# CU-Production/simple_mmd_renderer

Hardware: AMD Instinct MI355X
Metric: skinned vertices/sec (instance-sharded crowd); achieved HBM GB/s vs roofline (higher is better)
Workload: dtype f32

## Files before the change

simple_mmd_renderer_amd/csrc/kernels.hip:

```cpp
#include "instance_list.hpp"
#include "kernels.hpp"
#include "motion_blend.hpp"
#include "motion_clock.hpp"

#include <type_traits>
#ifdef PK_STAMPS
#include <algorithm>
#include <cstdio>
#include <vector>
#endif

#ifdef MMDX_FAST_MATH
#pragma clang fp contract(fast)
#define MMDX_K(name) name##_fast
#else
#define MMDX_K(name) name
#endif

#if (defined(PK_SKIP_WALK) || defined(PK_SKIP_SKIN) || defined(FUSED4_SKIP_WALK) || defined(PK_STAMPS)) && !defined(MMDX_DIAGNOSTIC_BUILD)
#error "PK_SKIP_* / FUSED4_SKIP_WALK / PK_STAMPS are timing diagnostics (wrong results): add MMDX_DIAGNOSTIC_BUILD to MMDX_BUILD_DEFS"
#endif

namespace mmdx {
namespace {
// ... 14 lines not shown
#define MMDX_STORE_POLICY 1
#endif
#if MMDX_STORE_POLICY != 0 && MMDX_STORE_POLICY != 1
#error "MMDX_STORE_POLICY: 0 (plain) or 1 (nt); the inline-asm sc0/sc1 flavours of round 3 corrupted data and no longer exist"
#endif
#ifndef MMDX_WALK_ZPAIR
#define MMDX_WALK_ZPAIR 1
#endif
typedef float v4f __attribute__((ext_vector_type(4)));
__device__ __forceinline__ void store16(float4 *dst, const float4 v) {
#if MMDX_STORE_POLICY == 1
    __builtin_nontemporal_store(v4f{v.x, v.y, v.z, v.w}, reinterpret_cast<v4f *>(dst));
#else
    *dst = v;
#endif
}
__device__ __forceinline__ void store3(float *dst, float x, float y, float z) {
#if MMDX_STORE_POLICY == 1
    __builtin_nontemporal_store(x, dst); __builtin_nontemporal_store(y, dst + 1); __builtin_nontemporal_store(z, dst + 2);
#else
    dst[0] = x; dst[1] = y; dst[2] = z;
#endif
}
template <typename T>
__device__ __forceinline__ void store_elem(T *dst, const T v) {
#if MMDX_STORE_POLICY == 1
    __builtin_nontemporal_store(v, dst);
#else
    *dst = v;
#endif
}

typedef float v2f __attribute__((ext_vector_type(2)));

struct M12 {
    v2f p0, p1, p2, p3;
    v2f q0, q1;
};

__device__ __forceinline__ M12 load_m12(const float4 *P, uint32_t b) {
    const float4 A = P[b], B = P[b + 1], C = P[b + 2];
    M12 m;
    m.p0 = v2f{A.x, A.y}; m.p1 = v2f{A.z, A.w};
    m.p2 = v2f{B.x, B.y}; m.p3 = v2f{B.z, B.w};
    m.q0 = v2f{C.x, C.y}; m.q1 = v2f{C.z, C.w};
    return m;
}
__device__ __forceinline__ M12 blend2(const M12 &a, const M12 &b, float s1, float l) {
    M12 r;
    r.p0 = a.p0 * s1 + b.p0 * l; r.p1 = a.p1 * s1 + b.p1 * l;
    r.p2 = a.p2 * s1 + b.p2 * l; r.p3 = a.p3 * s1 + b.p3 * l;
    r.q0 = a.q0 * s1 + b.q0 * l; r.q1 = a.q1 * s1 + b.q1 * l;
    return r;
}
__device__ __forceinline__ M12 mul_add(const M12 &a, float wa, const M12 &b, float wb) {
    M12 r;
    r.p0 = a.p0 * wa + b.p0 * wb; r.p1 = a.p1 * wa + b.p1 * wb;
    r.p2 = a.p2 * wa + b.p2 * wb; r.p3 = a.p3 * wa + b.p3 * wb;
    r.q0 = a.q0 * wa + b.q0 * wb; r.q1 = a.q1 * wa + b.q1 * wb;
    return r;
}
__device__ __forceinline__ M12 add_mul(const M12 &t, const M12 &c, float wc) {
    M12 r;
    r.p0 = t.p0 + c.p0 * wc; r.p1 = t.p1 + c.p1 * wc;
    r.p2 = t.p2 + c.p2 * wc; r.p3 = t.p3 + c.p3 * wc;
    r.q0 = t.q0 + c.q0 * wc; r.q1 = t.q1 + c.q1 * wc;
    return r;
}
__device__ __forceinline__ void xform_pos(const M12 &m, v2f xy, float z, v2f &oxy, float &oz) {
    oxy = ((m.p0 * xy.x + m.p1 * xy.y) + m.p2 * z) + m.p3;
    const v2f t = m.q0 * xy;
    oz = ((t.x + t.y) + z * m.q1.x) + m.q1.y;
}
__device__ __forceinline__ void xform_nrm(const M12 &m, v2f xy, float z, v2f &oxy, float &oz) {
    oxy = (m.p0 * xy.x + m.p1 * xy.y) + m.p2 * z;
    const v2f t = m.q0 * xy;
    oz = (t.x + t.y) + z * m.q1.x;
}

template <typename T>
__device__ __forceinline__ void copy_chunk(const unsigned char *img, T *g, uint32_t q, uint32_t shift,
                                           uint32_t n, bool aligned16) {
    constexpr uint32_t EPC = 16 / sizeof(T);
    const uint32_t lo = q * EPC;
    if (aligned16 && lo >= shift && lo + EPC <= shift + n) {
        const float4 v = *reinterpret_cast<const float4 *>(img + size_t(q) * 16);
        store16(reinterpret_cast<float4 *>(g + lo), v);
    } else {
        const T *l = reinterpret_cast<const T *>(img);
#pragma unroll
        for (uint32_t e = 0; e < EPC; ++e) {
            const uint32_t i = lo + e;
            if (i >= shift && i < shift + n) store_elem(g + i, l[i]);
        }
    }
}

template <int THREADS, typename TA, typename TB>
__device__ __forceinline__ void copy_out2(const unsigned char *imgA, TA *outA, size_t baseA,
                                          uint32_t shA, uint32_t nA, const unsigned char *imgB,
                                          TB *outB, size_t baseB, uint32_t shB, uint32_t nB,
                                          bool aligned16, int tid) {
    const uint32_t ncA = (shA + nA + 16 / sizeof(TA) - 1) / (16 / sizeof(TA));
    const uint32_t ncB = (shB + nB + 16 / sizeof(TB) - 1) / (16 / sizeof(TB));
    TA *gA = outA + baseA - shA;
    TB *gB = outB + baseB - shB;
    for (uint32_t q = tid; q < ncA + ncB; q += THREADS) {
        if (q < ncA) copy_chunk<TA>(imgA, gA, q, shA, nA, aligned16);
        else copy_chunk<TB>(imgB, gB, q - ncA, shB, nB, aligned16);
    }
}


template <int THREADS, int CA, int CB, int I, bool WT = false>
struct CopyFast {
    static __device__ __forceinline__ void run(const unsigned char *img, uint32_t gapB, float4 *outA,
                                               float4 *outB, int tid) {
        constexpr int TOTAL = CA + CB;
        if constexpr (I * THREADS < TOTAL) {
            constexpr bool full = (I + 1) * THREADS <= TOTAL;
            const int q = tid + I * THREADS;
            const bool inA = (I + 1) * THREADS <= CA ? true : (I * THREADS >= CA ? false : q < CA);
            float4 v = make_float4(0.f, 0.f, 0.f, 0.f);
            if (full || q < TOTAL)
                v = *reinterpret_cast<const float4 *>(img + (inA ? 0u : gapB - uint32_t(CA) * 16u) +
                                                      size_t(q) * 16);
            CopyFast<THREADS, CA, CB, I + 1, WT>::run(img, gapB, outA, outB, tid);
            if (full || q < TOTAL) {
                if constexpr (WT) {
                    typedef unsigned int v4u __attribute__((ext_vector_type(4)));
                    constexpr int kSc1Nt = 2 | 16;
                    const v4u d = {__float_as_uint(v.x), __float_as_uint(v.y), __float_as_uint(v.z), __float_as_uint(v.w)};
                    if (inA) {
                        const __amdgpu_buffer_rsrc_t r = __builtin_amdgcn_make_buffer_rsrc(outA, 0, uint32_t(CA) * 16u, 0x00027000);
                        __builtin_amdgcn_raw_buffer_store_b128(d, r, uint32_t(q) * 16u, 0, kSc1Nt);
                    } else {
                        const __amdgpu_buffer_rsrc_t r = __builtin_amdgcn_make_buffer_rsrc(outB, 0, uint32_t(CB) * 16u, 0x00027000);
                        __builtin_amdgcn_raw_buffer_store_b128(d, r, uint32_t(q - CA) * 16u, 0, kSc1Nt);
                    }
                } else {
                    float4 *dst = inA ? outA + q : outB + (q - CA);
                    store16(dst, v);
                }
            }
        }
    }
};
template <int THREADS, int CA, int CB, bool WT = false>
__device__ __forceinline__ void copy_out_fast(const unsigned char *img, uint32_t gapB, float4 *outA,
                                              float4 *outB, int tid) {
    CopyFast<THREADS, CA, CB, 0, WT>::run(img, gapB, outA, outB, tid);
}

struct Slot {
    v2f pxy, nxy, uv;
    float pz, nz;
    float w0, w1, w2, w3;
    uint32_t b0, b1, b2, b3;
    uint32_t perm;
    uint32_t rb, rlen;
    int cls;
    bool act;
};

template <bool F16>
struct RawEntry { using type = float4; };
template <>
struct RawEntry<true> { using type = uint2; };

constexpr uint32_t kRowAhead = 4;

template <bool F16, uint32_t B = kRowAhead>
struct RowHead {
    typename RawEntry<F16>::type e[B];
};
template <bool F16>
__device__ __forceinline__ typename RawEntry<F16>::type row_entry(const void *entries, uint32_t base, uint32_t j) {
    using Raw = typename RawEntry<F16>::type;
    const uint32_t off = (base + j * 64u) * uint32_t(sizeof(Raw));
    return *reinterpret_cast<const Raw *>(static_cast<const unsigned char *>(entries) + off);
}
template <bool F16, uint32_t B = kRowAhead>
__device__ __forceinline__ void row_prefetch(const void *entries, uint32_t base, uint32_t len, RowHead<F16, B> &h) {
    using Raw = typename RawEntry<F16>::type;
    const uint32_t last = len ? len - 1 : 0u;
#pragma unroll
    for (uint32_t i = 0; i < B; ++i) {
        Raw v = Raw{};
        if (len) v = row_entry<F16>(entries, base, min(i, last));
        h.e[i] = v;
    }
}
template <bool F16, uint32_t B = kRowAhead, typename Body>
__device__ __forceinline__ void row_consume(const void *entries, uint32_t base, uint32_t len, const RowHead<F16, B> &h,
                                            Body body) {
    using Raw = typename RawEntry<F16>::type;
    auto apply = [&](const Raw r) {
        if constexpr (F16) {
            body(h2f(r.x & 0xffffu), h2f(r.x >> 16), h2f(r.y & 0xffffu), uint32_t(r.y >> 16));
        } else {
            body(r.x, r.y, r.z, __float_as_uint(r.w));
        }
    };
    if (len == 0) return;
    const uint32_t last = len - 1;
    Raw cur[B], nxt[B];
#pragma unroll
    for (uint32_t i = 0; i < B; ++i) cur[i] = h.e[i];
    for (uint32_t j = 0; j < len; j += B) {
#pragma unroll
        for (uint32_t i = 0; i < B; ++i) nxt[i] = cur[i];
        if (j + B < len) {
#pragma unroll
            for (uint32_t i = 0; i < B; ++i) nxt[i] = row_entry<F16>(entries, base, min(j + B + i, last));
        }
#pragma unroll
        for (uint32_t i = 0; i < B; ++i)
            if (i == 0 || j + i < len) apply(cur[i]);
#pragma unroll
        for (uint32_t i = 0; i < B; ++i) cur[i] = nxt[i];
    }
}
template <bool F16, uint32_t B = kRowAhead, typename Body>
__device__ __forceinline__ void for_row(const void *entries, uint32_t base, uint32_t len, Body body) {
    RowHead<F16, B> h;
    row_prefetch<F16, B>(entries, base, len, h);
    row_consume<F16, B>(entries, base, len, h, body);
}

#ifndef MMDX_WALK_DEPTH32
#define MMDX_WALK_DEPTH32 4
#endif
#ifndef MMDX_WALK_DEPTH16
#define MMDX_WALK_DEPTH16 4
#endif
template <bool F16>
struct WalkHead {
    static constexpr uint32_t D = F16 ? MMDX_WALK_DEPTH16 : MMDX_WALK_DEPTH32;
    typename RawEntry<F16>::type e[D];
};
template <bool F16>
__device__ __forceinline__ void walk_head(const void *entries, uint32_t base, uint32_t len, WalkHead<F16> &h) {
    using Raw = typename RawEntry<F16>::type;
    const uint32_t last = len ? len - 1 : 0u;
#pragma unroll
    for (uint32_t i = 0; i < WalkHead<F16>::D; ++i) h.e[i] = len ? row_entry<F16>(entries, base, min(i, last)) : Raw{};
}
template <bool F16, typename Body>
__device__ __forceinline__ void walk_from_head(const void *entries, uint32_t base, uint32_t len, WalkHead<F16> &h, Body body) {
    using Raw = typename RawEntry<F16>::type;
    constexpr uint32_t D = WalkHead<F16>::D;
    if (len == 0) return;
    auto apply = [&](const Raw r) {
        if constexpr (F16) body(h2f(r.x & 0xffffu), h2f(r.x >> 16), h2f(r.y & 0xffffu), uint32_t(r.y >> 16));
        else body(r.x, r.y, r.z, __float_as_uint(r.w));
    };
    const uint32_t last = len - 1;
    uint32_t j = 0;
    for (; j + D < len; j += D) {
#pragma unroll
        for (uint32_t i = 0; i < D; ++i) {
            apply(h.e[i]);
            h.e[i] = row_entry<F16>(entries, base, min(j + D + i, last));
        }
    }
#pragma unroll
    for (uint32_t i = 0; i < D; ++i)
        if (i == 0 || j + i < len) apply(h.e[i]);
}
template <bool F16, typename Body>
__device__ __forceinline__ void walk_rolling(const void *entries, uint32_t base, uint32_t len, Body body) {
    WalkHead<F16> h;
    walk_head<F16>(entries, base, len, h);
    walk_from_head<F16>(entries, base, len, h, body);
}

__device__ __forceinline__ float slot_weight(const float *rates, const uint32_t *slot_top,
                                             const uint32_t *chain_off, const float *chain_rate,
                                             uint32_t s) {
    float r = rates[slot_top[s]];
    bool skip = r < kMorphEps;
    for (uint32_t c = chain_off[s]; !skip && c < chain_off[s + 1]; ++c) {
        r = chain_rate[c] * r;
        skip = r < kMorphEps;
    }
    return skip ? 0.f : r;
}

__device__ __forceinline__ bool map_workgroup(const DeformParams &p, uint32_t &tile, uint32_t &grp) {
    const uint32_t xcd = blockIdx.x & 7u, k = blockIdx.x >> 3;
    const uint32_t T = p.ntiles >> 3, main_count = T * p.ngroups;
    if (k < main_count) {
        grp = k / T;
        tile = xcd * T + (k - grp * T);
        return true;
    }
    const uint32_t r = xcd * p.rem_per_xcd + (k - main_count);
    if (r >= (p.ntiles & 7u) * p.ngroups) return false;
    const uint32_t rt = r / p.ngroups;
    tile = 8u * T + rt;
    grp = r - rt * p.ngroups;
    return true;
}

template <int LAYOUT, int MORPH, bool F16>
__device__ __forceinline__ void load_slot(const DeformParams &p, const TileHdr &th, uint32_t s, Slot &q) {
// ... 87 lines not shown
    const bool flat = p.fused_rates == nullptr;
    auto row_src = [&](uint32_t e, uint32_t bone) {
        const uint32_t g = gcount == 1 ? 0u : e / nb4;
        uint32_t inst = inst0 + g * istep;
        if constexpr (SEL) {
            inst = p.sel_ids[inst];
            if (inst >= p.ni) inst = 0u;
        }
        return reinterpret_cast<const float4 *>(p.palettes + size_t(inst) * p.nb * 16 + size_t(bone) * 16 + (e & 3u) * 4);
    };
    auto row_put = [&](uint32_t e, const float4 row) {
        const uint32_t g = gcount == 1 ? 0u : e / nb4, rem = e - g * nb4, lb = rem >> 2, r = rem & 3u;
        float *en = reinterpret_cast<float *>(pal + size_t(g) * p.pal_stride) + lb * 12;
        *reinterpret_cast<float2 *>(en + (r >> 1) * 4 + (r & 1u) * 2) = make_float2(row.x, row.y);
        en[8 + r] = row.z;
    };
    auto chain = [&](float r, uint32_t c0, uint32_t c1) {
        bool skip = r < kMorphEps;
        for (uint32_t c = c0; !skip && c < c1; ++c) {
            r = p.chain_rate[c] * r;
            skip = r < kMorphEps;
        }
        return skip ? 0.f : r;
    };

#pragma unroll
    for (int k = 0; k < VPT; ++k) load_slot<LAYOUT, MORPH, F16>(p, th, slot_base + uint32_t(tid) + uint32_t(k) * THREADS, sl[k]);
    uint32_t bone[kPalBatch];
#pragma unroll
    for (int i = 0; i < kPalBatch; ++i) {
        const uint32_t e = uint32_t(tid) + uint32_t(i) * THREADS;
        bone[i] = e < rows ? bones[((gcount == 1 ? e : e % nb4)) >> 2] : 0u;
    }
    uint32_t top[kWgtBatch], c0[kWgtBatch], c1[kWgtBatch];
    float wv[kWgtBatch];
#pragma unroll
    for (int i = 0; i < kWgtBatch; ++i) {
        const uint32_t sidx = uint32_t(tid) + uint32_t(i) * THREADS;
        top[i] = c0[i] = c1[i] = 0u;
        wv[i] = 0.f;
        if (kWalk && sidx < ns) {
            if (flat) wv[i] = p.wslot[sidx];
            else { top[i] = p.slot_top[sidx]; c0[i] = p.chain_off[sidx]; c1[i] = p.chain_off[sidx + 1]; }
        }
    }
    if constexpr (kWalk) {
#pragma unroll
        for (int k = 0; k < VPT; ++k) row_prefetch<F16, BH>(p.entries, sl[k].rb, sl[k].rlen, hd[k]);
    }
    float4 row[kPalBatch];
#pragma unroll
    for (int i = 0; i < kPalBatch; ++i) {
        const uint32_t e = uint32_t(tid) + uint32_t(i) * THREADS;
        row[i] = e < rows ? *row_src(e, bone[i]) : make_float4(0.f, 0.f, 0.f, 0.f);
    }
    if (kWalk && !flat) {
#pragma unroll
        for (int i = 0; i < kWgtBatch; ++i)
            if (uint32_t(tid) + uint32_t(i) * THREADS < ns) wv[i] = p.fused_rates[top[i]];
    }
#pragma unroll
    for (int i = 0; i < kPalBatch; ++i) {
        const uint32_t e = uint32_t(tid) + uint32_t(i) * THREADS;
        if (e < rows) row_put(e, row[i]);
    }
    if constexpr (kWalk) {
#pragma unroll
        for (int i = 0; i < kWgtBatch; ++i) {
            const uint32_t sidx = uint32_t(tid) + uint32_t(i) * THREADS;
            if (sidx <= ns) wl[sidx] = sidx < ns ? (flat ? wv[i] : chain(wv[i], c0[i], c1[i])) : 0.f;
        }
    }
    for (uint32_t e = uint32_t(kPalBatch) * THREADS + uint32_t(tid); e < rows; e += THREADS)
        row_put(e, *row_src(e, bones[(e % nb4) >> 2]));
    if constexpr (kWalk) {
        for (uint32_t sidx = uint32_t(kWgtBatch) * THREADS + uint32_t(tid); sidx <= ns; sidx += THREADS)
            wl[sidx] = sidx < ns ? (flat ? p.wslot[sidx] : slot_weight(p.fused_rates, p.slot_top, p.chain_off, p.chain_rate, sidx)) : 0.f;
    }
}

__device__ __forceinline__ M12 skin_matrix(const Slot &q, const float4 *P) {
    M12 m;
    if (q.cls == 0) {
        m = load_m12(P, q.b0);
    } else if (q.cls == 1) {
        const M12 a = load_m12(P, q.b1), e = load_m12(P, q.b0);
        const float l = q.w0;
        m = blend2(a, e, 1.0f - l, l);
        const bool lo = l < kLerpLo, hi = l > kLerpHi;
        if (__builtin_amdgcn_ballot_w64(lo || hi) != 0) {
            if (lo) m = a;
            else if (hi) m = e;
        }
    } else {
        {
            const M12 a = load_m12(P, q.b0), b = load_m12(P, q.b1);
            m = mul_add(a, q.w0, b, q.w1);
        }
        __builtin_amdgcn_sched_barrier(0);
        {
            const M12 c = load_m12(P, q.b2);
            m = add_mul(m, c, q.w2);
        }
        __builtin_amdgcn_sched_barrier(0);
        {
            const M12 d = load_m12(P, q.b3);
            m = add_mul(m, d, q.w3);
        }
    }
    return m;
}

template <bool MAX>
__device__ __forceinline__ float bound_op(float a, float b) { return MAX ? fmaxf(a, b) : fminf(a, b); }
__device__ __forceinline__ int f2key(float x) { const int b = __float_as_int(x); return b ^ ((b >> 31) & 0x7fffffff); }
__device__ __forceinline__ float key2f(int k) { return __int_as_float(k ^ ((k >> 31) & 0x7fffffff)); }
template <bool MAX>
__device__ __forceinline__ int key_op(int a, int b) { return MAX ? max(a, b) : min(a, b); }
template <int CTRL>
__device__ __forceinline__ int dpp_i(int v) { return __builtin_amdgcn_mov_dpp(v, CTRL, 0xf, 0xf, false); }
template <int CTRL>
__device__ __forceinline__ void dpp_step6(int (&k)[6]) {
#pragma unroll
    for (int c = 0; c < 6; ++c) k[c] = c < 3 ? key_op<false>(k[c], dpp_i<CTRL>(k[c])) : key_op<true>(k[c], dpp_i<CTRL>(k[c]));
}
__device__ __forceinline__ float wave_bounds6(const float (&mn)[3], const float (&mx)[3], uint32_t lane) {
    int k[6];
#pragma unroll
    for (int c = 0; c < 3; ++c) {
        k[c] = mn[c] != mn[c] ? INT_MAX : f2key(mn[c]);
        k[3 + c] = mx[c] != mx[c] ? INT_MIN : f2key(mx[c]);
    }
    dpp_step6<0xb1>(k);
    dpp_step6<0x4e>(k);
    dpp_step6<0x141>(k);
    dpp_step6<0x140>(k);
    int r[6];
#pragma unroll
    for (int c = 0; c < 6; ++c) {
        const int a = __builtin_amdgcn_readlane(k[c], 0), b = __builtin_amdgcn_readlane(k[c], 16);
        const int d = __builtin_amdgcn_readlane(k[c], 32), e = __builtin_amdgcn_readlane(k[c], 48);
        r[c] = c < 3 ? key_op<false>(key_op<false>(a, b), key_op<false>(d, e)) : key_op<true>(key_op<true>(a, b), key_op<true>(d, e));
    }
    const int s = lane == 0 ? r[0] : lane == 1 ? r[1] : lane == 2 ? r[2] : lane == 3 ? r[3] : lane == 4 ? r[4] : r[5];
    return s == (lane < 3 ? INT_MAX : INT_MIN) ? __builtin_nanf("") : key2f(s);
}

struct BoundsOut {
    float *lds;
    float *out;
};

struct NoHook { __device__ __forceinline__ void operator()() const {} };
template <int THREADS, int LAYOUT, int VPT, bool TILE, bool ALL_FAST, bool WT = false, bool BOUNDS = false, typename Hook = NoHook>
__device__ __forceinline__ void skin_instance(const DeformParams &p, const Slot (&sl)[VPT], const float4 *P,
                                              unsigned char *img, uint32_t inst, uint32_t v0, uint32_t nvt,
                                              const v2f (&cxy)[VPT], const float (&cz)[VPT], int tid, Hook after_barrier = Hook(),
                                              BoundsOut bo = BoundsOut{nullptr, nullptr}) {
    const size_t vbase = size_t(inst) * p.pitch + v0;
    const bool al = p.out_aligned != 0;
    const uint32_t sh4 = al ? uint32_t((vbase * 3) & 3) : 0u;
    const uint32_t sh8 = al ? uint32_t((vbase * 3) & 7) : 0u;
    float bmn[3], bmx[3];
    if constexpr (BOUNDS) {
#pragma unroll
        for (int c = 0; c < 3; ++c) bmn[c] = bmx[c] = __builtin_nanf("");
    }
#pragma unroll
    for (int k = 0; k < VPT; ++k) {
        const Slot &q = sl[k];
        if (!q.act) continue;
        const M12 m = skin_matrix(q, P);
        v2f oxy, rxy;
        float oz, rz;
        xform_pos(m, cxy[k], cz[k], oxy, oz);
        xform_nrm(m, q.nxy, q.nz, rxy, rz);
        oxy = oxy * p.pos_scale;
        oz = oz * p.pos_scale;
        if constexpr (BOUNDS) {
            float w[3] = {oxy.x, oxy.y, oz};
            if constexpr (LAYOUT == MMDX_OUT_SOA_POS16) {
#pragma unroll
                for (int c = 0; c < 3; ++c) w[c] = h2f(f2h(w[c]));
            }
#pragma unroll
            for (int c = 0; c < 3; ++c) { bmn[c] = bound_op<false>(bmn[c], w[c]); bmx[c] = bound_op<true>(bmx[c], w[c]); }
        }
        if constexpr (TILE) {
            const size_t v = vbase + uint32_t(tid) + uint32_t(k) * THREADS;
            if constexpr (LAYOUT == MMDX_OUT_SOA) {
                float *A = reinterpret_cast<float *>(p.out_a) + v * 3, *B = reinterpret_cast<float *>(p.out_b) + v * 3;
                store3(A, oxy.x, oxy.y, oz);
                store3(B, rxy.x, rxy.y, rz);
            } else if constexpr (LAYOUT == MMDX_OUT_VERTEX32) {
                float *A = reinterpret_cast<float *>(p.out_a) + v * 8;
                if (al) {
                    store16(reinterpret_cast<float4 *>(A), make_float4(oxy.x, oxy.y, oz, rxy.x));
                    store16(reinterpret_cast<float4 *>(A) + 1, make_float4(rxy.y, rz, q.uv.x, q.uv.y));
                } else {
                    A[0] = oxy.x; A[1] = oxy.y; A[2] = oz; A[3] = rxy.x; A[4] = rxy.y; A[5] = rz; A[6] = q.uv.x; A[7] = q.uv.y;
                }
            } else {
                unsigned short *A = reinterpret_cast<unsigned short *>(p.out_a) + v * 3;
                float *B = reinterpret_cast<float *>(p.out_b) + v * 3;
                A[0] = f2h(oxy.x); A[1] = f2h(oxy.y); A[2] = f2h(oz);
                B[0] = rxy.x; B[1] = rxy.y; B[2] = rz;
            }
            continue;
        }
        if constexpr (LAYOUT == MMDX_OUT_SOA) {
            float *A = reinterpret_cast<float *>(img) + sh4 + q.perm * 3;
            float *B = reinterpret_cast<float *>(img + kSoaImgBytes) + sh4 + q.perm * 3;
            A[0] = oxy.x; A[1] = oxy.y; A[2] = oz;
            B[0] = rxy.x; B[1] = rxy.y; B[2] = rz;
        } else if constexpr (LAYOUT == MMDX_OUT_VERTEX32) {
            float4 *I = reinterpret_cast<float4 *>(img) + q.perm * 2;
            I[0] = make_float4(oxy.x, oxy.y, oz, rxy.x);
            I[1] = make_float4(rxy.y, rz, q.uv.x, q.uv.y);
        } else {
            unsigned short *A = reinterpret_cast<unsigned short *>(img) + sh8 + q.perm * 3;
            float *B = reinterpret_cast<float *>(img + kP16ImgBytes) + sh4 + q.perm * 3;
            A[0] = f2h(oxy.x); A[1] = f2h(oxy.y); A[2] = f2h(oz);
            B[0] = rxy.x; B[1] = rxy.y; B[2] = rz;
        }
    }
    if constexpr (BOUNDS) {
        const uint32_t lane = uint32_t(tid) & 63u, wave = uint32_t(tid) >> 6;
        const float v = wave_bounds6(bmn, bmx, lane);
        if (lane < 6) (TILE ? bo.out : bo.lds)[wave * 6 + lane] = v;
    }
    if constexpr (TILE) return;
    __syncthreads();
    after_barrier();
    if constexpr (BOUNDS) {
        if (tid < 6) {
            float r = bo.lds[tid];
#pragma unroll
            for (int w = 1; w < THREADS / 64; ++w)
                r = tid < 3 ? bound_op<false>(r, bo.lds[w * 6 + tid]) : bound_op<true>(r, bo.lds[w * 6 + tid]);
            bo.out[tid] = r;
        }
    }
    const bool fast = ALL_FAST || (al && nvt == kTileVerts && sh4 == 0 && sh8 == 0);
    if constexpr (LAYOUT == MMDX_OUT_SOA) {
        float *oa = reinterpret_cast<float *>(p.out_a), *ob = reinterpret_cast<float *>(p.out_b);
        if (fast)
            copy_out_fast<THREADS, kTileVerts * 12 / 16, kTileVerts * 12 / 16, WT>(
                img, kSoaImgBytes, reinterpret_cast<float4 *>(oa + vbase * 3),
                reinterpret_cast<float4 *>(ob + vbase * 3), tid);
        else
            copy_out2<THREADS, float, float>(img, oa, vbase * 3, sh4, nvt * 3, img + kSoaImgBytes, ob,
                                             vbase * 3, sh4, nvt * 3, al, tid);
    } else if constexpr (LAYOUT == MMDX_OUT_VERTEX32) {
        float *oa = reinterpret_cast<float *>(p.out_a);
        if (fast)
            copy_out_fast<THREADS, kTileVerts * 32 / 16, 0>(
                img, 0u, reinterpret_cast<float4 *>(oa + vbase * 8), nullptr, tid);
        else
            copy_out2<THREADS, float, float>(img, oa, vbase * 8, 0u, nvt * 8, img, oa, 0, 0u, 0u, al,
                                             tid);
    } else {
        unsigned short *oa = reinterpret_cast<unsigned short *>(p.out_a);
        float *ob = reinterpret_cast<float *>(p.out_b);
        if (fast)
            copy_out_fast<THREADS, kTileVerts * 6 / 16, kTileVerts * 12 / 16>(
                img, kP16ImgBytes, reinterpret_cast<float4 *>(oa + vbase * 3),
                reinterpret_cast<float4 *>(ob + vbase * 3), tid);
        else
            copy_out2<THREADS, unsigned short, float>(img, oa, vbase * 3, sh8, nvt * 3,
                                                      img + kP16ImgBytes, ob, vbase * 3, sh4, nvt * 3,
                                                      al, tid);
    }
}

__device__ __forceinline__ void stagger_start(const DeformParams &p) {
    if (p.stagger == 0u || p.slots_per_cu < 2u) return;
    const uint32_t round = blockIdx.x >> 8;
    if (round >= p.slots_per_cu) return;
    for (uint32_t k = 0; k < round * p.stagger; k += 100) __builtin_amdgcn_s_sleep(100);
}

#ifndef MMDX_WALK_ROLLING
#define MMDX_WALK_ROLLING 1
#endif
#ifndef MMDX_WALK_PREFETCH
#define MMDX_WALK_PREFETCH 0
#endif
template <bool F16, bool ROLLING, typename Body>
__device__ __forceinline__ void fused4_walk(const void *entries, uint32_t rb, uint32_t rlen, Body body) {
    if constexpr (ROLLING && MMDX_WALK_ROLLING != 0) walk_rolling<F16>(entries, rb, __builtin_amdgcn_readfirstlane(rlen), body);
    else for_row<F16>(entries, rb, rlen, body);
}

template <int THREADS, int LAYOUT, int MORPH_MODE, bool F16, bool TILE, bool WT = false, bool BOUNDS = false>
__global__ __launch_bounds__(THREADS) void deform_kernel(const DeformParams p) {
    constexpr int MORPH = MORPH_MODE & 3;
    constexpr bool SELECT = (MORPH_MODE & kMorphSelect) != 0;
    constexpr int VPT = int(kTileVerts) / THREADS;
    extern __shared__ __attribute__((aligned(16))) unsigned char smem[];
    const int tid = threadIdx.x;
    uint32_t tile, grp;
    if (!map_workgroup(p, tile, grp)) return;
    if constexpr (MORPH == kMorphFused4) stagger_start(p);
    const TileHdr &th = p.tiles[tile];
    const uint32_t v0 = th.v0, nvt = th.nv;
    const bool ilv = (MORPH == kMorphNone || MORPH == kMorphShared || MORPH == kMorphFused1) &&
                     (SELECT ? p.sel_interleave != 0 : p.interleave != 0);
    const uint32_t inst0 = ilv ? grp : grp * p.group;
    const uint32_t istep = ilv ? p.ngroups : 1u;
    uint32_t gcount;
    if constexpr (SELECT) {
        const uint32_t nlive = p.sel_count ? min(uniform_u32(p.sel_count), p.sel_n) : p.sel_n;
        const uint32_t end = min(inst0 + p.group, nlive);
        gcount = ilv ? min(p.group, (nlive + p.ngroups - 1u - grp) / p.ngroups)
                     : (end > inst0 ? end - inst0 : 0u);
    } else {
        gcount = ilv ? (p.ni > grp ? min(p.group, (p.ni - grp + p.ngroups - 1) / p.ngroups) : 0u)
                     : min(p.group, p.ni - inst0);
    }
    if constexpr (SELECT) {
        if (gcount == 0 && !(MORPH == kMorphFused1 && grp == 0 && p.morphed)) return;
    }
    float4 *pal = reinterpret_cast<float4 *>(smem);
    unsigned char *stage = smem + p.stage_off;
    constexpr uint32_t kStage = stage_bytes(LAYOUT);

    Slot sl[VPT];
    constexpr uint32_t BH = MORPH == kMorphFused1 ? (F16 ? 16u : 8u) : kRowAhead;
    RowHead<F16, BH> hd[VPT];
    constexpr int kQuads = VPT == 1 ? 2 : 1, kPack = 4 * kQuads;
    const uint32_t wstride = p.ns + 1, wcount = uint32_t(kQuads) * wstride;
    auto pack_weight = [&](uint32_t g0, uint32_t i) {
        const float4 *src = reinterpret_cast<const float4 *>(p.wslot) + size_t((inst0 + g0) / 4) * wstride;
        return (i < wstride || g0 + 4 < gcount) ? src[i] : make_float4(0.f, 0.f, 0.f, 0.f);
    };
    if constexpr (MORPH == kMorphFused1) {
        setup_fused1<THREADS, LAYOUT, kMorphFused1, F16, VPT, BH, SELECT>(p, th, pal, reinterpret_cast<float *>(smem + p.w_off), inst0, istep,
                                                                   gcount, tid, 0u, sl, hd);
    } else {
        stage_palettes<THREADS, SELECT>(p, th, pal, inst0, istep, gcount, tid);
        if constexpr (MORPH == kMorphFused4) {
            float4 *wq0 = reinterpret_cast<float4 *>(smem + p.w_off);
            for (uint32_t i = tid; i < wcount && gcount; i += THREADS) wq0[i] = pack_weight(0, i);
        }
#pragma unroll
        for (int k = 0; k < VPT; ++k) load_slot<LAYOUT, MORPH, F16>(p, th, uint32_t(tid) + uint32_t(k) * THREADS, sl[k]);
    }
    __syncthreads();

    uint32_t buf = 0;
    constexpr uint32_t kAlignVerts = LAYOUT == MMDX_OUT_SOA_POS16 ? 8u : (LAYOUT == MMDX_OUT_SOA ? 4u : 1u);
    const bool all_fast = !TILE && p.out_aligned != 0 && nvt == kTileVerts && p.pitch % kAlignVerts == 0 && v0 % kAlignVerts == 0;
    auto instances = [&](auto all_fast_tag) {
    constexpr bool kAllFast = decltype(all_fast_tag)::value;
    auto run_instance = [&](uint32_t g, const v2f (&cxy)[VPT], const float (&cz)[VPT], auto hook) {
        uint32_t sel_inst = 0u;
        if constexpr (SELECT) {
            sel_inst = uniform_u32(p.sel_ids + (inst0 + g * istep));
            if (sel_inst >= p.ni) {
                hook();
                return;
            }
        }
        BoundsOut bo{nullptr, nullptr};
        if constexpr (BOUNDS) {
            constexpr uint32_t kUnits = TILE ? uint32_t(THREADS) / 64u : 1u;
            bo.lds = reinterpret_cast<float *>(smem + p.bounds_off) + buf * 48u;
            bo.out = p.bounds + (size_t(inst0 + g * istep) * p.ntiles + tile) * kUnits * 6u;
        }
        if constexpr (SELECT)
            skin_instance<THREADS, LAYOUT, VPT, TILE, kAllFast, WT, BOUNDS>(p, sl, pal + size_t(g) * p.pal_stride, stage + buf * kStage,
                                                                       sel_inst, v0, nvt, cxy, cz, tid, hook, bo);
        else
        skin_instance<THREADS, LAYOUT, VPT, TILE, kAllFast, WT, BOUNDS>(p, sl, pal + size_t(g) * p.pal_stride, stage + buf * kStage,
                                                                   inst0 + g * istep, v0, nvt, cxy, cz, tid, hook, bo);
        buf ^= 1u;
    };

    if constexpr (MORPH == kMorphNone || MORPH == kMorphShared) {
        v2f cxy[VPT];
        float cz[VPT];
#pragma unroll
        for (int k = 0; k < VPT; ++k) { cxy[k] = sl[k].pxy; cz[k] = sl[k].pz; }
        for (uint32_t g = 0; g < gcount; ++g) run_instance(g, cxy, cz, NoHook{});
    } else if constexpr (MORPH == kMorphFused1) {
        const float *wl = reinterpret_cast<const float *>(smem + p.w_off);
        v2f cxy[VPT];
        float cz[VPT];
#pragma unroll
        for (int k = 0; k < VPT; ++k) {
            v2f dxy = v2f{0.f, 0.f};
            float dz = 0.f;
            row_consume<F16, BH>(p.entries, sl[k].rb, sl[k].rlen, hd[k], [&](float ox, float oy, float oz, uint32_t slot) {
                const float w = wl[slot];
                if (!(w < kMorphEps)) { dxy = dxy + v2f{ox, oy} * w; dz = dz + oz * w; }
            });
            cxy[k] = sl[k].pxy + dxy; cz[k] = sl[k].pz + dz;
            if (k == 0 && grp == 0 && tile == 0 && tid == 0 && p.morphed && p.morph_seen) p.morph_seen[kSeenValid] = 0u;
            if (grp == 0 && p.morphed && sl[k].act) {
                float *mo = p.morphed + (size_t(v0) + uint32_t(tid) + uint32_t(k) * THREADS) * 3;
                mo[0] = cxy[k].x; mo[1] = cxy[k].y; mo[2] = cz[k];
            }
        }
        for (uint32_t g = 0; g < gcount; ++g) run_instance(g, cxy, cz, NoHook{});
    } else {
        float4 *wq = reinterpret_cast<float4 *>(smem + p.w_off);
        const bool wreg = wcount <= uint32_t(THREADS);
        constexpr bool kHead = VPT == 1 && !TILE && MMDX_WALK_ROLLING != 0 && MMDX_WALK_PREFETCH != 0;
        WalkHead<F16> head;
        const uint32_t hlen = __builtin_amdgcn_readfirstlane(sl[0].rlen);
        if constexpr (kHead) walk_head<F16>(p.entries, sl[0].rb, hlen, head);
        for (uint32_t g0 = 0; g0 < gcount;) {
            v2f dxy[VPT][kPack];
            float dz[VPT][kPack];
#pragma unroll
            for (int k = 0; k < VPT; ++k) {
#pragma unroll
                for (int j = 0; j < kPack; ++j) { dxy[k][j] = v2f{0.f, 0.f}; dz[k][j] = 0.f; }
                auto weights = [&](uint32_t slot, float (&w)[kPack]) {
                    const float4 a4 = wq[slot];
                    w[0] = a4.x; w[1] = a4.y; w[2] = a4.z; w[3] = a4.w;
                    if constexpr (kQuads == 2) {
                        const float4 b4 = wq[wstride + slot];
                        w[4] = b4.x; w[5] = b4.y; w[6] = b4.z; w[7] = b4.w;
                    }
                };
                auto walk = [&](auto body) {
                    if constexpr (kHead) walk_from_head<F16>(p.entries, sl[k].rb, hlen, head, body);
                    else fused4_walk<F16, !TILE>(p.entries, sl[k].rb, sl[k].rlen, body);
                };
#ifdef FUSED4_SKIP_WALK
                if (false) {
#else
                if (p.finite_offsets) {
#endif
                    walk([&](float ox, float oy, float oz, uint32_t slot) {
                        float w[kPack];
                        weights(slot, w);
                        const v2f oxy = v2f{ox, oy};
#if MMDX_WALK_ZPAIR
                        const v2f ozz = v2f{oz, oz};
#pragma unroll
                        for (int j = 0; j < kPack; j += 2) {
                            dxy[k][j] += oxy * w[j]; dxy[k][j + 1] += oxy * w[j + 1];
                            const v2f zz = v2f{dz[k][j], dz[k][j + 1]} + ozz * v2f{w[j], w[j + 1]};
                            dz[k][j] = zz.x; dz[k][j + 1] = zz.y;
                        }
#else
#pragma unroll
                        for (int j = 0; j < kPack; ++j) { dxy[k][j] += oxy * w[j]; dz[k][j] += oz * w[j]; }
#endif
                    });
                } else {
#ifndef FUSED4_SKIP_WALK
                    walk([&](float ox, float oy, float oz, uint32_t slot) {
                        float w[kPack];
                        weights(slot, w);
                        const v2f oxy = v2f{ox, oy};
#pragma unroll
                        for (int j = 0; j < kPack; ++j)
                            if (!(w[j] < kMorphEps)) { dxy[k][j] += oxy * w[j]; dz[k][j] += oz * w[j]; }
                    });
#endif
                }
            }
            const bool more = g0 + kPack < gcount;
            float4 wnext = make_float4(0.f, 0.f, 0.f, 0.f);
            if (more && wreg && uint32_t(tid) < wcount) wnext = pack_weight(g0 + kPack, uint32_t(tid));
            auto one = [&](int j, auto hook) {
                v2f cxy[VPT];
                float cz[VPT];
#pragma unroll
                for (int k = 0; k < VPT; ++k) {
                    cxy[k] = sl[k].pxy + dxy[k][j]; cz[k] = sl[k].pz + dz[k][j];
                }
                run_instance(g0 + j, cxy, cz, hook);
            };
#pragma unroll
            for (int j = 0; j + 1 < kPack; ++j)
                if (g0 + j < gcount) one(j, NoHook{});
            if (!more) {
                if (g0 + kPack - 1 < gcount) one(kPack - 1, NoHook{});
                break;
            }
            if constexpr (kHead) one(kPack - 1, [&]() {
                uint32_t rb = sl[0].rb;
                asm volatile("" : "+v"(rb));
                walk_head<F16>(p.entries, rb, hlen, head);
            });
            else one(kPack - 1, NoHook{});
            {
                if constexpr (TILE) __syncthreads();
                if (wreg) {
                    if (uint32_t(tid) < wcount) wq[tid] = wnext;
                } else {
                    for (uint32_t i = tid; i < wcount; i += THREADS) wq[i] = pack_weight(g0 + kPack, i);
                }
                __syncthreads();
            }
            g0 += kPack;
        }
    }
    };
    if constexpr (MORPH == kMorphFused1) {
        instances(std::false_type{});
    } else {
        if (all_fast) instances(std::true_type{});
        else instances(std::false_type{});
    }
}


constexpr int kPkThreads = 512;

struct PackSlot {
    v2f pxy, nxy;
    float pz, nz;
    float w0, w1, w2, w3;
    uint32_t b01, b23;
    uint32_t meta;
};
__device__ __forceinline__ PackSlot pack_slot(const Slot &q) {
    PackSlot s;
    s.pxy = q.pxy; s.nxy = q.nxy; s.pz = q.pz; s.nz = q.nz;
    s.w0 = q.w0; s.w1 = q.w1; s.w2 = q.w2; s.w3 = q.w3;
    s.b01 = q.b0 | (q.b1 << 16); s.b23 = q.b2 | (q.b3 << 16);
    s.meta = q.perm | (uint32_t(q.cls) << 10) | (q.act ? 1u << 12 : 0u);
    return s;
}
__device__ __forceinline__ M12 skin_matrix_packed(uint32_t cls, uint32_t b01, uint32_t b23, float w0, float w1, float w2, float w3,
                                                  const float4 *P) {
    M12 m;
    if (cls == 0) {
        m = load_m12(P, b01 & 0xffffu);
    } else if (cls == 1) {
        const M12 a = load_m12(P, b01 >> 16), e = load_m12(P, b01 & 0xffffu);
        m = blend2(a, e, 1.0f - w0, w0);
        const bool lo = w0 < kLerpLo, hi = w0 > kLerpHi;
        if (__builtin_amdgcn_ballot_w64(lo || hi) != 0) {
            if (lo) m = a;
            else if (hi) m = e;
        }
    } else {
        {
            const M12 a = load_m12(P, b01 & 0xffffu), b = load_m12(P, b01 >> 16);
            m = mul_add(a, w0, b, w1);
        }
        __builtin_amdgcn_sched_barrier(0);
        {
            const M12 c = load_m12(P, b23 & 0xffffu);
            m = add_mul(m, c, w2);
        }
        __builtin_amdgcn_sched_barrier(0);
        {
            const M12 d = load_m12(P, b23 >> 16);
            m = add_mul(m, d, w3);
        }
    }
    return m;
}

#ifndef PK_WAVES
#define PK_WAVES 6
#endif
template <int LAYOUT, bool F16, bool FIN>
__global__ __launch_bounds__(kPkThreads, PK_WAVES) void pack_kernel(const DeformParams p) {
    static_assert(LAYOUT == MMDX_OUT_SOA || LAYOUT == MMDX_OUT_SOA_POS16, "two output arrays");
    static_assert(kTileVerts == 512, "one sorted slot per lane");
    using Raw = typename RawEntry<F16>::type;
    extern __shared__ __attribute__((aligned(16))) unsigned char smem[];
    const int tid = threadIdx.x;
    uint32_t tile, grp;
    if (!map_workgroup(p, tile, grp)) return;
    const TileHdr &th = p.tiles[tile];
    const uint32_t v0 = th.v0, nvt = th.nv;
    const bool ilv = p.interleave != 0;
    const uint32_t nquads = (p.ni + 3u) >> 2, qstep = ilv ? p.ngroups : 1u;
    const uint32_t quad0 = ilv ? grp : grp * (p.group >> 2);
    const uint32_t npacks = quad0 < nquads ? min(p.group >> 2, (nquads - quad0 + qstep - 1) / qstep) : 0u;
    const uint32_t gcount = npacks * kPkPack;
    auto first_instance = [&](uint32_t g0) { return (quad0 + (g0 >> 2) * qstep) * 4u; };
    stagger_start(p);
    float4 *pal = reinterpret_cast<float4 *>(smem);
    float4 *wq = reinterpret_cast<float4 *>(smem + p.w_off);
    unsigned char *mp = smem + p.mp_off;
    unsigned char *imgB = smem + p.stage_off;
    const uint32_t wstride = p.ns + 1;
    auto pack_weight = [&](uint32_t g0, uint32_t i) {
        return reinterpret_cast<const float4 *>(p.wslot)[size_t(quad0 + (g0 >> 2) * qstep) * wstride + i];
    };
    const uint2 sl2 = p.ell[(v0 + uint32_t(tid)) >> 6];
    const uint32_t rbase = sl2.x + (uint32_t(tid) & 63u);
    const uint32_t rlen = __builtin_amdgcn_readfirstlane(sl2.y);
    const uint32_t last = rlen ? rlen - 1 : 0u;
    Raw e[4];
    auto row_head = [&]() {
        uint32_t rb = rbase;
        asm volatile("" : "+v"(rb));
#pragma unroll
        for (uint32_t i = 0; i < 4; ++i) e[i] = rlen ? row_entry<F16>(p.entries, rb, min(i, last)) : Raw{};
    };

    stage_palettes<kPkThreads>(p, th, pal, quad0 * 4u, 1u, gcount, tid, qstep);
    __builtin_amdgcn_sched_barrier(0);
    for (uint32_t i = tid; i < wstride; i += kPkThreads) wq[i] = pack_weight(0, i);
    __builtin_amdgcn_sched_barrier(0);
    PackSlot ps;
    {
        Slot q;
        load_slot<LAYOUT, kMorphFused4, F16>(p, th, uint32_t(tid), q);
        ps = pack_slot(q);
    }
    __builtin_amdgcn_sched_barrier(0);
    row_head();
    const bool wreg = wstride <= uint32_t(kPkThreads);
    constexpr uint32_t kAlignVerts = LAYOUT == MMDX_OUT_SOA_POS16 ? 8u : 4u;
    const bool al = p.out_aligned != 0;
    const bool fast = al && nvt == kTileVerts && p.pitch % kAlignVerts == 0 && v0 % kAlignVerts == 0;
    __syncthreads();

#ifdef PK_STAMPS
    unsigned long long st_acc[6] = {0, 0, 0, 0, 0, 0}, st_t = __builtin_amdgcn_s_memtime();
    const unsigned long long st_begin = st_t;
#define PK_STAMP(k) do { const unsigned long long n_ = __builtin_amdgcn_s_memtime(); st_acc[k] += n_ - st_t; st_t = n_; } while (0)
#else
#define PK_STAMP(k) do { } while (0)
#endif
    uint32_t buf = 0;
    for (uint32_t g0 = 0; g0 < gcount; g0 += kPkPack) {
        PK_STAMP(0);
        v2f axy[kPkPack], az01 = v2f{0.f, 0.f}, az23 = v2f{0.f, 0.f};
#pragma unroll
        for (uint32_t j = 0; j < kPkPack; ++j) axy[j] = v2f{0.f, 0.f};
        auto apply = [&](const Raw r) {
            float ox, oy, oz;
            uint32_t slot;
            if constexpr (F16) {
                ox = h2f(r.x & 0xffffu); oy = h2f(r.x >> 16); oz = h2f(r.y & 0xffffu); slot = r.y >> 16;
            } else {
                ox = r.x; oy = r.y; oz = r.z; slot = __float_as_uint(r.w);
            }
            const float4 w = wq[slot];
            const v2f oxy = v2f{ox, oy}, ozz = v2f{oz, oz};
            if constexpr (FIN) {
                axy[0] += oxy * w.x; axy[1] += oxy * w.y; axy[2] += oxy * w.z; axy[3] += oxy * w.w;
                az01 += ozz * v2f{w.x, w.y};
                az23 += ozz * v2f{w.z, w.w};
            } else {
                const v2f t0 = axy[0] + oxy * w.x, t1 = axy[1] + oxy * w.y, t2 = axy[2] + oxy * w.z, t3 = axy[3] + oxy * w.w;
                const v2f u01 = az01 + ozz * v2f{w.x, w.y}, u23 = az23 + ozz * v2f{w.z, w.w};
                const bool k0 = w.x < kMorphEps, k1 = w.y < kMorphEps, k2 = w.z < kMorphEps, k3 = w.w < kMorphEps;
                axy[0] = k0 ? axy[0] : t0; axy[1] = k1 ? axy[1] : t1; axy[2] = k2 ? axy[2] : t2; axy[3] = k3 ? axy[3] : t3;
                az01 = v2f{k0 ? az01.x : u01.x, k1 ? az01.y : u01.y};
                az23 = v2f{k2 ? az23.x : u23.x, k3 ? az23.y : u23.y};
            }
        };
#ifdef PK_SKIP_WALK
        if (false) {
#else
        if (rlen) {
#endif
// ... 701 lines not shown
```

Before: 245.0 billion.

## Specialize crowd instance loop with uniform copy, strided pointers, unit-scale path

Adds a specialized ALL_FAST, non-tiled, 256-thread crowd loop. It replaces the per-instance copy-out address arithmetic with a wave-uniform compile-time copy (CopyUniform) that advances precomputed output pointers by a fixed stride. It also drops the per-slot active check and the alignment shift computations, and adds a path that skips the pos_scale multiply when scale is 1.0. The aim is to cut scalar and vector address math and cndmask selects in the inner instance loop, which is paid for with extra template instantiations and code size.

```diff
diff --git a/profiles/loop_trim/loop_tail_new.s b/profiles/loop_trim/loop_tail_new.s
--- /dev/null
+++ b/profiles/loop_trim/loop_tail_new.s
@@ -0,0 +1,63 @@
+	v_lshlrev_b32_e32 v100, 4, v109
+	s_addc_u32 s17, s17, 0
+	s_mov_b64 s[18:19], 0
+	s_mov_b32 s36, 0
+	v_mov_b32_e32 v89, 0
+	s_branch .LBB0_155
+.LBB0_154:
+	s_or_b64 exec, exec, s[20:21]
+	s_waitcnt lgkmcnt(2)
+	v_pk_mul_f32 v[22:23], v[80:81], v[18:19]
+	v_pk_mul_f32 v[24:25], v[82:83], v[20:21]
+	v_pk_mul_f32 v[18:19], v[18:19], v[72:73]
+	v_pk_add_f32 v[22:23], v[22:23], v[24:25]
+	s_waitcnt lgkmcnt(1)
+	v_pk_mul_f32 v[24:25], v[54:55], v[14:15]
+	v_pk_mul_f32 v[20:21], v[20:21], v[74:75]
+	v_pk_add_f32 v[22:23], v[22:23], v[24:25]
+	v_pk_add_f32 v[18:19], v[18:19], v[20:21]
+	v_pk_add_f32 v[16:17], v[16:17], v[22:23]
+	s_waitcnt lgkmcnt(0)
+	v_pk_mul_f32 v[22:23], v[52:53], v[10:11]
+	v_pk_mul_f32 v[10:11], v[10:11], v[56:57]
+	v_add_f32_e32 v22, v22, v23
+	v_mul_f32_e32 v23, v54, v12
+	v_pk_mul_f32 v[14:15], v[14:15], v[58:59]
+	v_add_f32_e32 v10, v10, v11
+	v_mul_f32_e32 v11, v12, v58
+	v_add_f32_e32 v22, v23, v22
+	v_pk_add_f32 v[14:15], v[18:19], v[14:15]
+	v_add_f32_e32 v10, v11, v10
+	v_lshl_add_u32 v11, v92, 2, s37
+	v_mov_b32_e32 v88, v90
+	v_add_f32_e32 v13, v13, v22
+	v_add_u32_e32 v12, 0x1810, v11
+	ds_write2_b32 v11, v16, v17 offset1:1
+	ds_write_b32 v11, v13 offset:8
+	ds_write2_b32 v12, v14, v15 offset1:1
+	ds_write_b32 v11, v10 offset:6168
+	s_waitcnt lgkmcnt(0)
+	s_barrier
+	s_xor_b32 s36, s36, 1
+	v_add_u32_e32 v14, s37, v88
+	s_add_i32 s37, s37, s31
+	ds_read_b128 v[10:13], v14
+	ds_read_b128 v[14:17], v14 offset:8208
+	v_add_u32_e32 v18, s37, v88
+	ds_read_b128 v[18:21], v18
+	v_lshl_add_u64 v[22:23], s[18:19], 0, v[88:89]
+	s_add_i32 s30, s30, s34
+	s_add_i32 s33, s33, -1
+	v_lshl_add_u64 v[24:25], s[16:17], 0, v[22:23]
+	s_add_u32 s18, s18, s29
+	s_waitcnt lgkmcnt(1)
+	global_store_dwordx4 v[24:25], v[14:17], off nt
+	s_addc_u32 s19, s19, s28
+	s_cmp_eq_u32 s33, 0
+	v_lshl_add_u64 v[14:15], s[14:15], 0, v[22:23]
+	s_waitcnt lgkmcnt(0)
+	global_store_dwordx4 v[14:15], v[18:21], off nt
+	v_lshl_add_u64 v[14:15], s[8:9], 0, v[22:23]
+	global_store_dwordx4 v[14:15], v[10:13], off nt
+	s_cbranch_scc1 .LBB0_181
+.LBB0_155:
diff --git a/profiles/loop_trim/loop_tail_parent.s b/profiles/loop_trim/loop_tail_parent.s
--- /dev/null
+++ b/profiles/loop_trim/loop_tail_parent.s
@@ -0,0 +1,70 @@
+.LBB194_123:
+	s_or_b64 exec, exec, s[24:25]
+	s_waitcnt lgkmcnt(2)
+	v_pk_mul_f32 v[22:23], v[82:83], v[18:19]
+	v_pk_mul_f32 v[24:25], v[72:73], v[20:21]
+	v_pk_mul_f32 v[18:19], v[18:19], v[86:87]
+	v_pk_add_f32 v[22:23], v[22:23], v[24:25]
+	s_waitcnt lgkmcnt(1)
+	v_pk_mul_f32 v[24:25], v[54:55], v[14:15]
+	v_pk_mul_f32 v[20:21], v[20:21], v[88:89]
+	v_pk_add_f32 v[22:23], v[22:23], v[24:25]
+	v_pk_add_f32 v[18:19], v[18:19], v[20:21]
+	v_pk_add_f32 v[16:17], v[16:17], v[22:23]
+	s_waitcnt lgkmcnt(0)
+	v_pk_mul_f32 v[22:23], v[52:53], v[10:11]
+	v_pk_mul_f32 v[10:11], v[10:11], v[56:57]
+	v_add_f32_e32 v22, v22, v23
+	v_mul_f32_e32 v23, v54, v12
+	v_add_f32_e32 v22, v23, v22
+	v_add_f32_e32 v10, v10, v11
+	v_mul_f32_e32 v11, v12, v58
+	v_add_f32_e32 v13, v13, v22
+	v_pk_mul_f32 v[14:15], v[14:15], v[58:59]
+	v_add_f32_e32 v12, v11, v10
+	v_pk_mul_f32 v[10:11], s[18:19], v[16:17]
+	v_lshl_add_u32 v16, v95, 2, s42
+	v_pk_add_f32 v[14:15], v[18:19], v[14:15]
+	v_mul_f32_e32 v13, s18, v13
+	v_add_u32_e32 v17, 0x1810, v16
+	ds_write2_b32 v16, v10, v11 offset1:1
+	ds_write_b32 v16, v13 offset:8
+	ds_write2_b32 v17, v14, v15 offset1:1
+	ds_write_b32 v16, v12 offset:6168
+.LBB194_124:
+	s_or_b64 exec, exec, s[22:23]
+	s_mul_i32 s23, s60, s34
+	s_mul_hi_u32 s22, s60, s34
+	s_add_u32 s24, s23, s36
+	s_addc_u32 s22, s22, 0
+	v_add_u32_e32 v14, s42, v74
+	v_add3_u32 v18, s42, v108, v98
+	s_waitcnt lgkmcnt(0)
+	s_barrier
+	s_mul_i32 s26, s22, 12
+	s_mul_hi_u32 s22, s24, 12
+	ds_read_b128 v[10:13], v14
+	ds_read_b128 v[14:17], v14 offset:8208
+	ds_read_b128 v[18:21], v18
+	s_add_i32 s23, s22, s26
+	s_mul_i32 s22, s24, 12
+	s_add_u32 s22, s28, s22
+	v_mad_u64_u32 v[22:23], s[24:25], s24, 12, v[0:1]
+	s_addc_u32 s23, s29, s23
+	v_add_u32_e32 v23, s26, v23
+	s_waitcnt lgkmcnt(1)
+	global_store_dwordx4 v[22:23], v[14:17], off offset:2048 nt
+	s_xor_b32 s41, s41, 1
+	s_add_i32 s37, s37, s40
+	v_lshl_add_u64 v[14:15], s[22:23], 0, v[70:71]
+	v_lshl_add_u64 v[16:17], v[22:23], 0, s[20:21]
+	s_add_i32 s33, s33, -1
+	s_add_i32 s60, s60, s61
+	v_cndmask_b32_e64 v15, v17, v15, s[12:13]
+	v_cndmask_b32_e64 v14, v16, v14, s[12:13]
+	s_cmp_eq_u32 s33, 0
+	s_waitcnt lgkmcnt(0)
+	global_store_dwordx4 v[14:15], v[18:21], off nt
+	global_store_dwordx4 v100, v[10:13], s[22:23] nt
+	s_cbranch_scc1 .LBB194_154
+.LBB194_125:
diff --git a/simple_mmd_renderer_amd/csrc/kernels.hip b/simple_mmd_renderer_amd/csrc/kernels.hip
--- a/simple_mmd_renderer_amd/csrc/kernels.hip
+++ b/simple_mmd_renderer_amd/csrc/kernels.hip
@@ -190,6 +190,53 @@
     CopyFast<THREADS, CA, CB, 0, WT>::run(img, gapB, outA, outB, tid);
 }
 
+#ifndef MMDX_LOOP_UNIFORM_COPY
+#define MMDX_LOOP_UNIFORM_COPY 1
+#endif
+#ifndef MMDX_LOOP_UNIT_SCALE
+#define MMDX_LOOP_UNIT_SCALE 1
+#endif
+
+constexpr int copy_chunks_a(int layout) { return int(kTileVerts) * (layout == MMDX_OUT_SOA ? 12 : (layout == MMDX_OUT_VERTEX32 ? 32 : 6)) / 16; }
+constexpr int copy_chunks_b(int layout) { return layout == MMDX_OUT_VERTEX32 ? 0 : int(kTileVerts) * 12 / 16; }
+template <int THREADS, int CA, int CB>
+struct CopyMid {
+    static constexpr bool kHas = CB > 0 && CA % THREADS != 0;
+    static constexpr int kStep = CA / THREADS;
+    static __device__ __forceinline__ bool in_a(uint32_t wave) { return wave * 64u + uint32_t(kStep * THREADS) < uint32_t(CA); }
+    static __device__ __forceinline__ unsigned char *base(unsigned char *pa, unsigned char *pb, bool mid_a) {
+        return mid_a ? pa + kStep * THREADS * 16 : pb - (CA - kStep * THREADS) * 16;
+    }
+};
+
+template <int THREADS, int CA, int CB, int I>
+struct CopyUniform {
+    static __device__ __forceinline__ void run(const unsigned char *img, uint32_t gapB, unsigned char *pa, unsigned char *pb,
+                                               unsigned char *pm, bool mid_a, uint32_t wave, uint32_t tid16) {
+        constexpr int TOTAL = CA + CB;
+        static_assert(CA % 64 == 0 && TOTAL % 64 == 0 && THREADS % 64 == 0, "a wave's chunks must lie in one image");
+        if constexpr (I * THREADS < TOTAL) {
+            using Mid = CopyMid<THREADS, CA, CB>;
+            constexpr bool kMid = Mid::kHas && Mid::kStep == I;
+            const bool on = (I + 1) * THREADS <= TOTAL ? true : wave * 64u + uint32_t(I * THREADS) < uint32_t(TOTAL);
+            const bool inA = kMid ? mid_a : I * THREADS < CA;
+            const uint32_t lofs = uint32_t(I * THREADS) * 16u + (inA ? 0u : gapB - uint32_t(CA) * 16u);
+            float4 v = make_float4(0.f, 0.f, 0.f, 0.f);
+            if (on) v = *reinterpret_cast<const float4 *>(img + lofs + tid16);
+            CopyUniform<THREADS, CA, CB, I + 1>::run(img, gapB, pa, pb, pm, mid_a, wave, tid16);
+            if (on) {
+                unsigned char *dst = kMid ? pm : (I * THREADS < CA ? pa + I * THREADS * 16 : pb + (I * THREADS - CA) * 16);
+                store16(reinterpret_cast<float4 *>(dst + tid16), v);
+            }
+        }
+    }
+};
+
+struct LoopForms {
+    uint32_t wave;
+    bool mid_a;
+};
+
 struct Slot {
     v2f pxy, nxy, uv;
     float pz, nz;
@@ -583,15 +630,18 @@
 };
 
 struct NoHook { __device__ __forceinline__ void operator()() const {} };
-template <int THREADS, int LAYOUT, int VPT, bool TILE, bool ALL_FAST, bool WT = false, bool BOUNDS = false, typename Hook = NoHook>
+template <int THREADS, int LAYOUT, int VPT, bool TILE, bool ALL_FAST, bool WT = false, bool BOUNDS = false, bool FORMS = false,
+          bool UNIT = false, typename Hook = NoHook>
 __device__ __forceinline__ void skin_instance(const DeformParams &p, const Slot (&sl)[VPT], const float4 *P,
                                               unsigned char *img, uint32_t inst, uint32_t v0, uint32_t nvt,
                                               const v2f (&cxy)[VPT], const float (&cz)[VPT], int tid, Hook after_barrier = Hook(),
-                                              BoundsOut bo = BoundsOut{nullptr, nullptr}) {
+                                              BoundsOut bo = BoundsOut{nullptr, nullptr}, const LoopForms *lf = nullptr,
+                                              unsigned char *pa = nullptr, unsigned char *pb = nullptr, unsigned char *pm = nullptr) {
+    static_assert(!FORMS || (ALL_FAST && !TILE), "the loop forms belong to the ALL_FAST loop");
     const size_t vbase = size_t(inst) * p.pitch + v0;
     const bool al = p.out_aligned != 0;
-    const uint32_t sh4 = al ? uint32_t((vbase * 3) & 3) : 0u;
-    const uint32_t sh8 = al ? uint32_t((vbase * 3) & 7) : 0u;
+    const uint32_t sh4 = FORMS ? 0u : (al ? uint32_t((vbase * 3) & 3) : 0u);
+    const uint32_t sh8 = FORMS ? 0u : (al ? uint32_t((vbase * 3) & 7) : 0u);
     float bmn[3], bmx[3];
     if constexpr (BOUNDS) {
 #pragma unroll
@@ -600,14 +650,19 @@
 #pragma unroll
     for (int k = 0; k < VPT; ++k) {
         const Slot &q = sl[k];
-        if (!q.act) continue;
+        if constexpr (!FORMS) {
+            if (!q.act) continue;
+        }
         const M12 m = skin_matrix(q, P);
         v2f oxy, rxy;
         float oz, rz;
         xform_pos(m, cxy[k], cz[k], oxy, oz);
         xform_nrm(m, q.nxy, q.nz, rxy, rz);
-        oxy = oxy * p.pos_scale;
-        oz = oz * p.pos_scale;
+        if constexpr (!UNIT) {
+            oxy = oxy * p.pos_scale;
+            oz = oz * p.pos_scale;
+            if constexpr (LAYOUT == MMDX_OUT_SOA_POS16) asm volatile("" : "+v"(oxy), "+v"(oz));
+        }
         if constexpr (BOUNDS) {
             float w[3] = {oxy.x, oxy.y, oz};
             if constexpr (LAYOUT == MMDX_OUT_SOA_POS16) {
@@ -673,6 +728,13 @@
         }
     }
     const bool fast = ALL_FAST || (al && nvt == kTileVerts && sh4 == 0 && sh8 == 0);
+    if constexpr (FORMS && !WT && MMDX_LOOP_UNIFORM_COPY != 0) {
+        uint32_t tid16 = uint32_t(tid) * 16u;
+        asm volatile("" : "+v"(tid16));
+        constexpr uint32_t kGapB = LAYOUT == MMDX_OUT_SOA ? kSoaImgBytes : (LAYOUT == MMDX_OUT_VERTEX32 ? 0u : kP16ImgBytes);
+        CopyUniform<THREADS, copy_chunks_a(LAYOUT), copy_chunks_b(LAYOUT), 0>::run(img, kGapB, pa, pb, pm, lf->mid_a, lf->wave, tid16);
+        return;
+    }
     if constexpr (LAYOUT == MMDX_OUT_SOA) {
         float *oa = reinterpret_cast<float *>(p.out_a), *ob = reinterpret_cast<float *>(p.out_b);
         if (fast)
@@ -782,8 +844,30 @@
     uint32_t buf = 0;
     constexpr uint32_t kAlignVerts = LAYOUT == MMDX_OUT_SOA_POS16 ? 8u : (LAYOUT == MMDX_OUT_SOA ? 4u : 1u);
     const bool all_fast = !TILE && p.out_aligned != 0 && nvt == kTileVerts && p.pitch % kAlignVerts == 0 && v0 % kAlignVerts == 0;
-    auto instances = [&](auto all_fast_tag) {
+    constexpr bool kCrowdForms = !TILE && THREADS == 256 && (MORPH == kMorphNone || MORPH == kMorphShared);
+    constexpr size_t kBytesA = LAYOUT == MMDX_OUT_SOA ? 12u : (LAYOUT == MMDX_OUT_VERTEX32 ? 32u : 6u), kBytesB = 12u;
+    auto instances = [&](auto all_fast_tag, auto unit_tag) {
     constexpr bool kAllFast = decltype(all_fast_tag)::value;
+    constexpr bool kForms = kCrowdForms && kAllFast;
+    constexpr bool kUnit = kForms && decltype(unit_tag)::value;
+    LoopForms lf{0u, false};
+    using Mid = CopyMid<THREADS, copy_chunks_a(LAYOUT), copy_chunks_b(LAYOUT)>;
+    unsigned char *pa = nullptr, *pb = nullptr, *pm = nullptr;
+    size_t step_a = 0, step_b = 0, step_m = 0;
+    if constexpr (kForms) {
+        lf.wave = __builtin_amdgcn_readfirstlane(uint32_t(tid) >> 6);
+        lf.mid_a = Mid::in_a(lf.wave);
+        if constexpr (!SELECT) {
+            const size_t vb = size_t(inst0) * p.pitch + v0;
+            pa = reinterpret_cast<unsigned char *>(p.out_a) + vb * kBytesA;
+            step_a = size_t(istep) * p.pitch * kBytesA;
+            if constexpr (copy_chunks_b(LAYOUT) != 0) {
+                pb = reinterpret_cast<unsigned char *>(p.out_b) + vb * kBytesB;
+                step_b = size_t(istep) * p.pitch * kBytesB;
+            }
+            if constexpr (Mid::kHas) { pm = Mid::base(pa, pb, lf.mid_a); step_m = lf.mid_a ? step_a : step_b; }
+        }
+    }
     auto run_instance = [&](uint32_t g, const v2f (&cxy)[VPT], const float (&cz)[VPT], auto hook) {
         uint32_t sel_inst = 0u;
         if constexpr (SELECT) {
@@ -799,7 +883,22 @@
             bo.lds = reinterpret_cast<float *>(smem + p.bounds_off) + buf * 48u;
             bo.out = p.bounds + (size_t(inst0 + g * istep) * p.ntiles + tile) * kUnits * 6u;
         }
-        if constexpr (SELECT)
+        if constexpr (kForms) {
+            if constexpr (SELECT) {
+                const size_t vb = size_t(sel_inst) * p.pitch + v0;
+                pa = reinterpret_cast<unsigned char *>(p.out_a) + vb * kBytesA;
+                if constexpr (copy_chunks_b(LAYOUT) != 0) pb = reinterpret_cast<unsigned char *>(p.out_b) + vb * kBytesB;
+                if constexpr (Mid::kHas) pm = Mid::base(pa, pb, lf.mid_a);
+            }
+            skin_instance<THREADS, LAYOUT, VPT, TILE, kAllFast, WT, BOUNDS, true, kUnit>(
+                p, sl, pal + size_t(g) * p.pal_stride, stage + buf * kStage, SELECT ? sel_inst : inst0 + g * istep, v0, nvt, cxy, cz,
+                tid, hook, bo, &lf, pa, pb, pm);
+            if constexpr (!SELECT) {
+                pa += step_a;
+                if constexpr (copy_chunks_b(LAYOUT) != 0) pb += step_b;
+                if constexpr (Mid::kHas) pm += step_m;
+            }
+        } else if constexpr (SELECT)
             skin_instance<THREADS, LAYOUT, VPT, TILE, kAllFast, WT, BOUNDS>(p, sl, pal + size_t(g) * p.pal_stride, stage + buf * kStage,
                                                                        sel_inst, v0, nvt, cxy, cz, tid, hook, bo);
         else
@@ -934,10 +1033,14 @@
     }
     };
     if constexpr (MORPH == kMorphFused1) {
-        instances(std::false_type{});
+        instances(std::false_type{}, std::false_type{});
+    } else if constexpr (kCrowdForms && MMDX_LOOP_UNIT_SCALE != 0) {
+        if (all_fast && p.pos_scale == 1.0f) instances(std::true_type{}, std::true_type{});
+        else if (all_fast) instances(std::true_type{}, std::false_type{});
+        else instances(std::false_type{}, std::false_type{});
     } else {
-        if (all_fast) instances(std::true_type{});
-        else instances(std::false_type{});
+        if (all_fast) instances(std::true_type{}, std::false_type{});
+        else instances(std::false_type{}, std::false_type{});
     }
 }
 
```

Result: no change. 246.9 billion, median of 6 (+0.8%).
